# ascentai/diy-gym

Measured on AMD Instinct MI355X. Metric: env steps/sec (whole node), higher is better.
Workload: dtype f32; 1 GPU; ur_high_5 x 16384 envs per GPU; envs_total=16384, substeps=2, auto_reset=True, launch=hipGraph replay of 8-step segments, parallelism=independent env shards x1, no collective, envs_per_wavefront=64, lds_bytes_per_workgroup=160512, parity=vs the C oracle only; parity with pybullet itself is UNPINNED (DESIGN.md 4)

## Files before the change

### diy_gym_amd/csrc/dg_solver.h

```cpp
#pragma once
#include "dg_kernels.h"
#include "dg_hull.h"

namespace dg {

enum { PS_UPDATE = 0, PS_KIN, PS_COLLIDE, PS_ABA, PS_MINV, PS_ROWS, PS_PGS, PS_INTEGRATE, PS_OUTPUT, PS_PGS_MOTOR, PS_PGS_LIMIT, PS_PGS_CONTACT, PS_COUNT,
       PS_ROW = PS_COUNT + 12  };
template <bool PROF> struct Prof;
template <> struct Prof<false> { DGD void start() {} DGD void stamp(int) {} };
template <> struct Prof<true> {
  unsigned long long last, acc[PS_COUNT];
  DGD void start() { _Pragma("unroll") for (int k = 0; k < PS_COUNT; k++) acc[k] = 0ull; last = __builtin_amdgcn_s_memtime(); }
  DGD void stamp(int id) {
    unsigned long long t = __builtin_amdgcn_s_memtime();
    _Pragma("unroll") for (int k = 0; k < PS_COUNT; k++) if (k == id) acc[k] += t - last;
    last = t;
  }
};

struct WShape { int type, body, glink; M3 R; V3 p; float prm0, prm1, prm2, mu; int poff, npts; };

template <int LANES>
DGD void shape_world(const Lane<LANES>& ln, int sh, WShape& o) {
  cip si = ln.sc.SI + sh * DG_SI_STRIDE; cfp sf = ln.sc.SF + sh * DG_SF_STRIDE;
// ... 1657 lines not shown
}

DGD float half_swap_max(float x) {
  float a = x, b = x;
  asm volatile("s_nop 1\n\tv_permlane32_swap_b32 %0, %1" : "+v"(a), "+v"(b));
  return fmaxf(a, b);
}
DGD float half_swap_sum(float x) {
  float a = x, b = x;
  asm volatile("s_nop 1\n\tv_permlane32_swap_b32 %0, %1" : "+v"(a), "+v"(b));
  return a + b;
}
template <int LANES>
DGD void pgs_reg_halves(const Lane<LANES>& ln, int wave) {
  constexpr int RN = 6;
  const DevScene& sc = ln.sc; const float h = sc.h; const float thr_abs = sqrtf(sc.HF[DG_HF_RESIDUAL_THRESHOLD]);
  const int lane = threadIdx.x & 63, half = lane >> 5, el = (lane & 31) + 32 * wave;
  float* const col = ln.lds - lane + el;
  const bool valid = (int)blockIdx.x * 64 + el < sc.num_envs;
  const int b0 = sc.reg_body[0], b1 = sc.helper_body;
  const int f0 = ln.bi(b0)[DG_BI_FIRST_LINK], f1 = ln.bi(b1)[DG_BI_FIRST_LINK], n0 = ln.bi(b0)[DG_BI_N_LINKS], n1 = ln.bi(b1)[DG_BI_N_LINKS];
  const int n = half ? n1 : n0, mvo = half ? ln.plb(b1)[PLB_MINV] : ln.plb(b0)[PLB_MINV], dvo = half ? ln.plb(b1)[PLB_DV] : ln.plb(b0)[PLB_DV];
  const int mo0 = half ? ln.pll(f1)[PLL_MROW] : ln.pll(f0)[PLL_MROW];
  auto W = [&](int slot) -> float& { return col[slot * 64]; };
  float rM[RN * RN], rdv[RN], rb[RN], racc[RN], rdi[RN], rdg[RN], smax[RN], lb[2][RN], la[2][RN]; bool any_limit = false;
  if (n0 == RN && n1 == RN) {
    const float* const cm = col + (size_t)mvo * 64; const float* const cr = col + (size_t)mo0 * 64;
#pragma unroll
    for (int i = 0; i < RN; i++) {
      const float mf0 = ln.mt.v[3 * (f0 + i) + 2], mf1 = ln.mt.v[3 * (f1 + i) + 2], maxf = half ? mf1 : mf0;
      smax[i] = maxf < 0.f ? -maxf : maxf * sc.hm;
#pragma unroll
      for (int c = 0; c < RN; c++) rM[i * RN + c] = cm[(i * RN + c) * 64];
      rb[i] = cr[(i * MR_STRIDE + MR_B) * 64]; rdg[i] = rM[i * RN + i]; rdi[i] = 1.0f / rdg[i];
      lb[0][i] = cr[(i * MR_STRIDE + MR_LO_B) * 64]; la[0][i] = cr[(i * MR_STRIDE + MR_LO_ACC) * 64];
      lb[1][i] = cr[(i * MR_STRIDE + MR_HI_B) * 64]; la[1][i] = cr[(i * MR_STRIDE + MR_HI_ACC) * 64];
      rdv[i] = 0.f; racc[i] = 0.f;
    }
  } else {
#pragma unroll
  for (int i = 0; i < RN; i++) {
    const bool has = i < n; const int ic = has ? i : 0;
    const float mf0 = ln.mt.v[3 * (f0 + (i < n0 ? i : 0)) + 2], mf1 = ln.mt.v[3 * (f1 + (i < n1 ? i : 0)) + 2];
    const float maxf = half ? mf1 : mf0;
    smax[i] = has ? (maxf < 0.f ? -maxf : maxf * sc.hm) : 0.f;
    const int mo = mo0 + ic * MR_STRIDE;
    rb[i] = has ? W(mo + MR_B) : 0.f; rdg[i] = has ? W(mvo + ic * n + ic) : 1.f; rdi[i] = has ? 1.0f / rdg[i] : 0.f;
    lb[0][i] = W(mo + MR_LO_B); la[0][i] = has ? W(mo + MR_LO_ACC) : -1.f;
    lb[1][i] = W(mo + MR_HI_B); la[1][i] = has ? W(mo + MR_HI_ACC) : -1.f;
    any_limit = any_limit || la[0][i] >= 0.f || la[1][i] >= 0.f;
    rdv[i] = 0.f; racc[i] = 0.f;
#pragma unroll
    for (int c = 0; c < RN; c++) { const bool hc = has && c < n; const float m = W(mvo + ic * n + (c < n ? c : 0)); rM[i * RN + c] = hc ? m : 0.f; }
  }
  }
  if (sc.HF[DG_HF_MOTOR_GUESS] > 0.f) chain_motor_guess(rM, rb, smax, racc, rdv, limit_ptol(sc), lb[0], la[0], lb[1], la[1]);
  unsigned lim_rows = 0u;
#pragma unroll
  for (int i = 0; i < RN; i++) { if (__any(la[0][i] >= 0.f)) lim_rows |= 1u << (2 * i); if (__any(la[1][i] >= 0.f)) lim_rows |= 2u << (2 * i); }
  (void)any_limit;
  constexpr int CM = DG_SPLIT_MAX_CONTACTS;
  const int ncont = (int)W(sc.cont_off), g = (half ? ln.plb(b1)[PLB_DV] : ln.plb(b0)[PLB_DV]) - sc.dv_base;
  int cmax = 0;
#pragma unroll
  for (int c = 0; c < CM; c++) if (__any(c < ncont)) cmax = c + 1;
  float cJ[3 * CM][RN], cR[3 * CM][RN], cb[3 * CM], cdg[3 * CM], cdi[3 * CM], cacc[3 * CM], cmu[CM];
  if (cmax > 0) {
    const int nt = sc.nt, rs = sc.crow_tail + 3;
#pragma unroll
    for (int c = 0; c < CM; c++) {
      const bool has = c < ncont; const int cc = has ? c : 0;
      cmu[c] = has ? W(sc.cont_off + 1 + cc * CL_STRIDE + CL_MU) : 0.f;
#pragma unroll
      for (int d = 0; d < 3; d++) {
        const int r = 3 * c + d, ro = sc.tr_off + (3 * cc + d) * rs;
#pragma unroll
        for (int k = 0; k < RN; k++) { const bool hk = has && k < n; const int kk = k < n ? k : 0; const float j = W(ro + g + kk), rr = W(ro + nt + g + kk); cJ[r][k] = hk ? j : 0.f; cR[r][k] = hk ? rr : 0.f; }
        const float bb = W(ro + 2 * nt), dd = W(ro + 2 * nt + 2);
        cb[r] = has ? bb : 0.f; cdg[r] = has ? dd : 1.f; cdi[r] = (has && dd > 1e-18f) ? frcp(dd) : 0.f;
        const float a0 = W(ro + 2 * nt + 1); cacc[r] = (has && cdi[r] != 0.f) ? a0 : 0.f;
#pragma unroll
        for (int k = 0; k < RN; k++) rdv[k] += cR[r][k] * cacc[r];
      }
    }
  }
  bool live = valid; int iters_done = 0;
  auto contact_row = [&](int r, float lo, float hi, float lv, float& maxabs) {
    float jp = 0.f;
#pragma unroll
    for (int k = 0; k < RN; k++) jp += cJ[r][k] * rdv[k];
    const float jv = half_swap_sum(jp);
    const float nacc = fminf(fmaxf(cacc[r] + (cb[r] - jv) * cdi[r], lo), hi);
    const float delta = cdi[r] != 0.f ? (nacc - cacc[r]) * lv : 0.f; cacc[r] += delta;
#pragma unroll
    for (int k = 0; k < RN; k++) rdv[k] += cR[r][k] * delta;
    maxabs = fmaxf(maxabs, fabsf(delta * cdg[r]));
  };
  auto sweep = [&](auto with_limits, auto with_contacts) {
    float maxabs = 0.f; const float lv = live ? 1.f : 0.f;
#pragma unroll
    for (int i = 0; i < RN; i++) {
      const float want = racc[i] + (rb[i] - rdv[i]) * rdi[i];
      const float nacc = __builtin_amdgcn_fmed3f(want, -smax[i], smax[i]);
      const float delta = (nacc - racc[i]) * lv; racc[i] += delta;
#pragma unroll
      for (int c = 0; c < RN; c++) rdv[c] += rM[i * RN + c] * delta;
      maxabs = fmaxf(maxabs, fabsf(delta * rdg[i]));
    }
    if constexpr (decltype(with_limits)::value) {
#pragma unroll
      for (int i = 0; i < RN; i++) {
#pragma unroll
        for (int side = 0; side < 2; side++) {
          if (!((lim_rows >> (2 * i + side)) & 1u)) continue;
          const float sg = side == 0 ? 1.f : -1.f; const bool act = la[side][i] >= 0.f;
          const float nacc = fmaxf(la[side][i] + (lb[side][i] - sg * rdv[i]) * rdi[i], 0.f);
          const float delta = act ? (nacc - la[side][i]) * lv : 0.f; la[side][i] += delta;
          const float sd = sg * delta;
#pragma unroll
          for (int c = 0; c < RN; c++) rdv[c] += rM[i * RN + c] * sd;
          maxabs = fmaxf(maxabs, fabsf(delta * rdg[i]));
        }
      }
    }
    if constexpr (decltype(with_contacts)::value) {
#pragma unroll
      for (int c = 0; c < CM; c++) if (c < cmax) contact_row(3 * c, 0.f, 3.0e38f, lv, maxabs);
#pragma unroll
      for (int c = 0; c < CM; c++) if (c < cmax) {
        const float lim = cmu[c] * cacc[3 * c];
        contact_row(3 * c + 1, -lim, lim, lv, maxabs); contact_row(3 * c + 2, -lim, lim, lv, maxabs);
      }
    }
    const float m = half_swap_max(maxabs);
    live = live && !(m <= thr_abs);
  };
  if (cmax > 0) {
    for (int it = 0; it < sc.iters; it++) { if (live) iters_done = it + 1; sweep(std::true_type{}, std::true_type{}); if (!__any(live)) break; }
  } else if (lim_rows == 0u) {
    for (int it = 0; it < sc.iters; it++) { if (live) iters_done = it + 1; sweep(std::false_type{}, std::false_type{}); if (!__any(live)) break; }
  } else {
    for (int it = 0; it < sc.iters; it++) { if (live) iters_done = it + 1; sweep(std::true_type{}, std::false_type{}); if (!__any(live)) break; }
  }
#pragma unroll
  for (int i = 0; i < RN; i++) if (i < n) { W(dvo + i) = rdv[i]; W(mo0 + i * MR_STRIDE + MR_ACC) = racc[i]; }
  if (cmax > 0 && half == 0) {
    const int rs = sc.crow_tail + 3;
#pragma unroll
    for (int c = 0; c < CM; c++) if (c < ncont) { _Pragma("unroll") for (int d = 0; d < 3; d++) W(sc.tr_off + (3 * c + d) * rs + sc.crow_tail + 1) = cacc[3 * c + d]; }
  }
  if (half == 0) W(split_slots(sc)) = (float)iters_done;
}

template <int LANES, bool PROF, bool PAR = false, bool SLICED = false, bool FULLWAVE = false>
DGD void substep(const Lane<LANES>& ln, int32_t* diag_out, Prof<PROF>& prof, float* smem = nullptr, float* gws = nullptr, int index = 0) {
  const DevScene& sc = ln.sc; const float h = sc.h; const int hb = PAR ? sc.helper_body : -1;
  const bool primary = SLICED ? (int)threadIdx.x < envs_per_wave(LANES) : true;
  constexpr int LCH = 6;
  int ncont = 0, wave_max_cont = 0, iters_done = 0;
  uint64_t limit_mask = 0ull;
  uint64_t limit_rows = 0ull;
  const float thr = sc.HF[DG_HF_RESIDUAL_THRESHOLD]; const int rs = crow_stride(sc.crow_tail);
  const bool early = PAR && sc.early_dyn && index == 0;
  constexpr int EPW = envs_per_wave(LANES), SLN = SLICED ? 64 / EPW : 1, SLOG = SLN == 64 ? 6 : SLN == 16 ? 4 : SLN == 8 ? 3 : SLN == 4 ? 2 : SLN == 2 ? 1 : 0;
  const int qlane = threadIdx.x & 63, qsl = qlane & (SLN - 1), qe = qlane >> SLOG;
  const int qenv = blockIdx.x * EPW + qe; const bool qvalid = qenv < sc.num_envs; const int qec = qvalid ? qenv : sc.num_envs - 1;
  const Lane<LANES> lq(sc, ln.mt, SLICED ? ln.lds - qlane + qe : ln.lds, SLICED ? ln.st - ln.env + qec : ln.st, SLICED ? qec : ln.env, SLICED ? qvalid : ln.valid);
  if (primary) {
  if (index == sc.substeps - 1 && !early) for (int b = 0; b < sc.nba; b++) if (b != hb) save_prev_velocities(ln, b);
  if (!early) for (int b = 0; b < sc.nba; b++) if (b != hb) ln.kinematics(b);
  }
  if (PAR) __syncthreads();
  prof.stamp(PS_KIN);
  if constexpr (SLICED) collide<LANES, 64, SLN>(lq, 0, 0x7fffffff, -1, qsl);
  const bool own_collide = !(PAR && sc.coll_wave);
  if (primary) {
  if constexpr (SLICED) ncont = (int)ln.L(sc.cont_off);
  else if (own_collide) ncont = collide<LANES, FULLWAVE ? 64 : (PAR ? 64 : 0)>(ln);
  prof.stamp(PS_COLLIDE);
  }
  if (!early) for (int b = 0; b < sc.nba; b++) {
    if (b == hb || (ln.fixed(b) && ln.bi(b)[DG_BI_N_LINKS] == 0)) continue;
    const int mslices = (SLICED && !ln.plb(b)[PLB_CHAIN] && !sc.no_minv_slices) ? ln.minv_slices(b, SLN) : 0;
    if (primary) { if (ln.plb(b)[PLB_CHAIN]) ln.template dynamics_chain<6>(b, prof); else ln.dynamics(b, prof, mslices > 0); }
    if constexpr (SLICED) { if (mslices > 0) { lq.minv_sliced(b, qsl, mslices, SLN); prof.stamp(4 ); } }
    if (primary) {
      const int dvo = ln.plb(b)[PLB_DV], nv = ln.plb(b)[PLB_NV];
      for (int k = 0; k < nv; k++) ln.L(dvo + k) = 0.f;
    }
  }
  if (primary) {
  if (PAR) __syncthreads();
  if (!own_collide) {
    ncont = (int)ln.L(sc.cont_off);
    if (sc.coll_split) {
      const int nb2 = (int)ln.L(sc.cont2_off);
      if (__any(nb2 > 0)) {
        for (int j = 0; j < sc.max_contacts; j++) {
          if (!__any(j < nb2)) break;
          if (j < nb2 && ncont + j < sc.max_contacts) {
            float* dst = ln.lds + (sc.cont_off + 1 + (ncont + j) * CL_STRIDE) * envs_per_wave(LANES);
#pragma unroll
            for (int k = 0; k < CL_KEY + 1; k++) dst[k * envs_per_wave(LANES)] = ln.L(sc.cont2_off + 1 + j * CL_STRIDE + k);
          }
        }
        ncont = min(ncont + nb2, sc.max_contacts); ln.L(sc.cont_off) = (float)ncont;
      }
    }
  }
  const bool helper_rows = PAR && sc.split_pgs;
  if (helper_rows) {
    const int hf = ln.bi(hb)[DG_BI_FIRST_LINK], hn = ln.bi(hb)[DG_BI_N_LINKS];
    setup_link_rows(ln, 0, hf, limit_mask, limit_rows); setup_link_rows(ln, hf + hn, sc.nl, limit_mask, limit_rows);
  } else setup_link_rows(ln, 0, sc.nl, limit_mask, limit_rows);
  for (int b = 0; b < sc.nba; b++) {
    if (ln.bi(b)[DG_BI_N_LINKS] == 0 || b == sc.reg_body[0] || b == sc.reg_body[1] || (helper_rows && b == hb)) continue;
    motor_guess(ln, b);
  }
  if (sc.ncons > 0) build_constraint_rows(ln);
  const bool vel_dense = sc.dense && sc.nt >= 1 && sc.reg_body[0] < 0;
  wave_max_cont = [&] { int m = ncont; for (int o = 32; o > 0; o >>= 1) m = max(m, __shfl_xor(m, o)); return m; }();
  if (vel_dense && wave_max_cont > 0)
    for (int b = 0; b < sc.nba; b++) if (!(ln.fixed(b) && ln.bi(b)[DG_BI_N_LINKS] == 0)) ln.gen_vel_store(b, ln.plb(b)[PLB_DV]);
  if constexpr (!SLICED) {
  for (int c = 0; c < wave_max_cont; c++) {
    const bool has = c < ncont; const int mypair = has ? (int)ln.L(sc.cont_off + 1 + c * CL_STRIDE + CL_PAIR) : -1;
    bool todo = has && !build_contact_rows_base(ln, c, has, vel_dense);
    if (!sc.no_chain_rows) todo = todo && !build_contact_rows_chains(ln, c, todo);
    while (__any(todo)) {
      const int leader = __ffsll((long long)__ballot(todo)) - 1;
      const int pair = __shfl(mypair, leader);
      const bool mine = todo && mypair == pair;
      build_contact_rows(ln, c, pair, mine, vel_dense);
      todo = todo && !mine;
    }
  }
  prof.stamp(PS_ROWS);
  }
  }
  if constexpr (SLICED) {
    constexpr int SL = SLN, CPI = SL >= 4 ? SL / 4 : SL;
    const int sl = qsl;
    const int ncq = __shfl(ncont, qe), wmc = __builtin_amdgcn_readfirstlane(wave_max_cont);
    const bool vd = sc.dense && sc.nt >= 1 && sc.reg_body[0] < 0;
    const int csub = SL >= 4 ? sl >> 2 : sl, d_lo = SL >= 4 ? (sl & 3) : 0, d_hi = SL >= 4 ? ((sl & 3) < 3 ? (sl & 3) + 1 : 0) : 3;
    for (int c0 = 0; c0 < wmc; c0 += CPI) {
      const int c = c0 + csub; const bool has = c < ncq && d_lo < d_hi;
      const int mypair = has ? (int)lq.L(sc.cont_off + 1 + c * CL_STRIDE + CL_PAIR) : -1;
      bool todo = has && !build_contact_rows_base(lq, c, has, vd, d_lo, d_hi);
      while (__any(todo)) {
        const int leader = __ffsll((long long)__ballot(todo)) - 1;
        const int pair = __shfl(mypair, leader);
        const bool mine = todo && mypair == pair;
        build_contact_rows(lq, c, pair, mine, vd, d_lo, d_hi);
        todo = todo && !mine;
      }
    }
    prof.stamp(PS_ROWS);
  }
  bool split_now = false;
  if constexpr (PAR) split_now = split_decide_main(ln, wave_max_cont, limit_mask, limit_rows);
  const bool all_dense = sc.dense && sc.nt >= 1 && sc.reg_body[0] < 0;
  if constexpr (SLICED) {
    wave_max_cont = __builtin_amdgcn_readfirstlane(wave_max_cont);
    limit_rows = ((uint64_t)(uint32_t)__builtin_amdgcn_readfirstlane((int)(limit_rows >> 32)) << 32) | (uint32_t)__builtin_amdgcn_readfirstlane((int)(uint32_t)limit_rows);
  }
  if (SLICED && all_dense) {
    const bool try_regs = sc.split_pgs != -1;
    if constexpr (SLICED && LANES == 1) {
      iters_done = pgs_wave_env<PROF>(lq, __builtin_amdgcn_readfirstlane(ncont), limit_rows, prof);
    } else if constexpr (SLICED && LANES == 4) {
      if (sc.nt <= 16) { if (!(try_regs && pgs_sliced_regs_dispatch<LANES, 16, PROF>(ln, ncont, wave_max_cont, limit_rows, prof, iters_done))) iters_done = pgs_dense_sliced<LANES, 16, PROF>(ln, ncont, wave_max_cont, limit_rows, prof); }
      else if (!(try_regs && pgs_sliced_regs_dispatch<LANES, 32, PROF>(ln, ncont, wave_max_cont, limit_rows, prof, iters_done))) iters_done = pgs_dense_sliced<LANES, 32, PROF>(ln, ncont, wave_max_cont, limit_rows, prof);
    } else if constexpr (SLICED && LANES > 0) {
      if (sc.nt <= 8) { if (!(try_regs && pgs_sliced_regs_dispatch<LANES, 8, PROF>(ln, ncont, wave_max_cont, limit_rows, prof, iters_done))) iters_done = pgs_dense_sliced<LANES, 8, PROF>(ln, ncont, wave_max_cont, limit_rows, prof); }
      else if (sc.nt <= 16) { if (!(try_regs && pgs_sliced_regs_dispatch<LANES, 16, PROF>(ln, ncont, wave_max_cont, limit_rows, prof, iters_done))) iters_done = pgs_dense_sliced<LANES, 16, PROF>(ln, ncont, wave_max_cont, limit_rows, prof); }
      else if (sc.nt <= 24) iters_done = pgs_dense_sliced<LANES, 24, PROF>(ln, ncont, wave_max_cont, limit_rows, prof);
      else iters_done = pgs_dense_sliced<LANES, 32, PROF>(ln, ncont, wave_max_cont, limit_rows, prof);
    } else if constexpr (SLICED) {
      if (sc.nt <= 8) iters_done = pgs_dense_sliced_global<LANES, 8, PROF>(ln, smem, gws, ncont, wave_max_cont, limit_rows, prof);
      else if (sc.nt <= 16) iters_done = pgs_dense_sliced_global<LANES, 16, PROF>(ln, smem, gws, ncont, wave_max_cont, limit_rows, prof);
      else if (sc.nt <= 24) iters_done = pgs_dense_sliced_global<LANES, 24, PROF>(ln, smem, gws, ncont, wave_max_cont, limit_rows, prof);
      else iters_done = pgs_dense_sliced_global<LANES, 32, PROF>(ln, smem, gws, ncont, wave_max_cont, limit_rows, prof);
    }
  } else if (PAR && split_now) {
    prof.stamp(PS_PGS_MOTOR);
    pgs_reg_halves(ln, 0);
    prof.stamp(PS_PGS_LIMIT);
    __syncthreads();
    prof.stamp(PS_PGS_CONTACT);
    iters_done = (int)ln.L(split_slots(sc));
  } else if (primary) {
  bool live = ln.valid;
  constexpr bool FW = FULLWAVE || PAR;
  if (all_dense || (sc.dense && (wave_max_cont > 0 || limit_mask != 0ull) && sc.nl <= 32)) {
    for (int k = 0; k < 2; k++) if (sc.reg_body[k] >= 0) motor_guess(ln, sc.reg_body[k]);
    if (sc.nt <= 8) iters_done = pgs_dense<LANES, 8, PROF, FW>(ln, ncont, wave_max_cont, limit_rows, prof);
    else if (sc.nt <= 16) iters_done = pgs_dense<LANES, 16, PROF, FW>(ln, ncont, wave_max_cont, limit_rows, prof);
    else if (sc.nt <= 24) iters_done = pgs_dense<LANES, 24, PROF, FW>(ln, ncont, wave_max_cont, limit_rows, prof);
    else iters_done = pgs_dense<LANES, 32, PROF, FW>(ln, ncont, wave_max_cont, limit_rows, prof);
  } else {
  constexpr int NBR = 2, RN = 6;
  float rM[NBR][RN * RN], rdv[NBR][RN], rb[NBR][RN], racc[NBR][RN], rdi[NBR][RN], rdg[NBR][RN]; float smax[NBR][RN]; int rn[NBR];
#pragma unroll
  for (int k = 0; k < NBR; k++) {
    const int b = sc.reg_body[k]; rn[k] = 0;
#pragma unroll
    for (int i = 0; i < RN; i++) { rdv[k][i] = 0.f; rb[k][i] = 0.f; racc[k][i] = 0.f; rdi[k][i] = 0.f; rdg[k][i] = 0.f; smax[k][i] = 0.f;
      _Pragma("unroll") for (int c = 0; c < RN; c++) rM[k][i * RN + c] = 0.f; }
    if (b >= 0) {
      const int n = ln.bi(b)[DG_BI_N_LINKS], first = ln.bi(b)[DG_BI_FIRST_LINK], mvo = ln.plb(b)[PLB_MINV], mo0 = ln.pll(first)[PLL_MROW];
      rn[k] = n;
#pragma unroll
      for (int i = 0; i < RN; i++) {
        rdv[k][i] = 0.f; rb[k][i] = 0.f; racc[k][i] = 0.f; rdi[k][i] = 0.f; rdg[k][i] = 0.f; smax[k][i] = 0.f;
        if (i < n) {
          const float maxf = ln.mt.v[3 * (first + i) + 2]; smax[k][i] = maxf < 0.f ? -maxf : maxf * sc.hm;
          rb[k][i] = ln.L(mo0 + i * MR_STRIDE + MR_B); rdg[k][i] = ln.L(mvo + i * n + i); rdi[k][i] = 1.0f / rdg[k][i];
        }
#pragma unroll
        for (int c = 0; c < RN; c++) rM[k][i * RN + c] = (i < n && c < n) ? ln.L(mvo + i * n + c) : 0.f;
      }
    }
  }
  auto regs_to_lds = [&](int k) { const int b = sc.reg_body[k]; if (b < 0) return; const int dvo = ln.plb(b)[PLB_DV];
    _Pragma("unroll") for (int i = 0; i < RN; i++) if (i < rn[k]) ln.L(dvo + i) = rdv[k][i]; };
  auto lds_to_regs = [&](int k) { const int b = sc.reg_body[k]; if (b < 0) return; const int dvo = ln.plb(b)[PLB_DV];
    _Pragma("unroll") for (int i = 0; i < RN; i++) if (i < rn[k]) rdv[k][i] = ln.L(dvo + i); };
  bool has_generic = false;
  for (int b = 0; b < sc.nba; b++) if (ln.bi(b)[DG_BI_N_LINKS] > 0 && b != sc.reg_body[0] && b != sc.reg_body[1]) has_generic = true;
  const float thr_abs = sqrtf(thr);
  if (sc.HF[DG_HF_MOTOR_GUESS] > 0.f) {
#pragma unroll
    for (int k = 0; k < NBR; k++) if (sc.reg_body[k] >= 0) {
      const int mo0 = ln.pll(ln.bi(sc.reg_body[k])[DG_BI_FIRST_LINK])[PLL_MROW]; const float ptol = limit_ptol(sc); const bool pinning = ptol >= 0.f;
      float lb0[RN], la0[RN], lb1[RN], la1[RN];
      _Pragma("unroll") for (int i = 0; i < RN; i++) { const bool has = i < rn[k]; const int mo = mo0 + (has ? i : 0) * MR_STRIDE;
        lb0[i] = ln.L(mo + MR_LO_B); la0[i] = has ? ln.L(mo + MR_LO_ACC) : -1.f; lb1[i] = ln.L(mo + MR_HI_B); la1[i] = has ? ln.L(mo + MR_HI_ACC) : -1.f; }
      chain_motor_guess(rM[k], rb[k], smax[k], racc[k], rdv[k], ptol, lb0, la0, lb1, la1);
      if (pinning) { _Pragma("unroll") for (int i = 0; i < RN; i++) if (i < rn[k]) { ln.L(mo0 + i * MR_STRIDE + MR_LO_ACC) = la0[i]; ln.L(mo0 + i * MR_STRIDE + MR_HI_ACC) = la1[i]; } }
    }
    if (has_generic) for (int b = 0; b < sc.nba; b++) {
      const int n = ln.bi(b)[DG_BI_N_LINKS]; if (n == 0 || b == sc.reg_body[0] || b == sc.reg_body[1]) continue;
      const int first = ln.bi(b)[DG_BI_FIRST_LINK], k0 = ln.fixed(b) ? 0 : 6, nv = ln.plb(b)[PLB_NV], dvo = ln.plb(b)[PLB_DV], mvo = ln.plb(b)[PLB_MINV];
      for (int i = 0; i < n; i++) { const int mo = ln.pll(first + i)[PLL_MROW]; const float a0 = ln.L(mo + MR_ACC) + fmaxf(ln.L(mo + MR_LO_ACC), 0.f) - fmaxf(ln.L(mo + MR_HI_ACC), 0.f); lds_axpy(ln, dvo, mvo + (k0 + i) * nv, a0, nv); }
    }
  }
  if (wave_max_cont > 0 && sc.warm_off >= 0) {
    const int nvm = sc.nv_max; const bool two = sc.crow_tail > 2 * nvm;
    regs_to_lds(0); regs_to_lds(1);
    for (int c = 0; c < wave_max_cont; c++) {
      const bool has = c < ncont; const int co = sc.cont_off + 1 + c * CL_STRIDE;
#pragma unroll
      for (int d = 0; d < 3; d++) {
        const int ro = sc.tr_off + (3 * c + d) * rs; const float a0 = has ? ln.L(ro + sc.crow_tail + 1) : 0.f;
        if (a0 != 0.f) {
          lds_axpy(ln, (int)ln.L(co + CL_DVA), ro + nvm, a0, nvm);
          if (two && (int)ln.L(co + CL_NVB) > 0) lds_axpy(ln, (int)ln.L(co + CL_DVB), ro + 3 * nvm, a0, nvm);
        }
      }
    }
    lds_to_regs(0); lds_to_regs(1);
  }
  for (int it = 0; it < sc.iters; it++) {
    float maxres = 0.f, maxabs = 0.f;
    {
      const float lv = live ? 1.f : 0.f;
#pragma unroll
      for (int i = 0; i < RN; i++) {
#pragma unroll
        for (int k = 0; k < NBR; k++) {
          const float want = racc[k][i] + (rb[k][i] - rdv[k][i]) * rdi[k][i];
          const float nacc = __builtin_amdgcn_fmed3f(want, -smax[k][i], smax[k][i]);
          const float delta = (nacc - racc[k][i]) * lv; racc[k][i] += delta;
#pragma unroll
          for (int c = 0; c < RN; c++) rdv[k][c] += rM[k][i * RN + c] * delta;
          maxabs = fmaxf(maxabs, fabsf(delta * rdg[k][i]));
        }
      }
    }
    if (has_generic) for (int b = 0; b < sc.nba; b++) {
      const int n = ln.bi(b)[DG_BI_N_LINKS]; if (n == 0 || b == sc.reg_body[0] || b == sc.reg_body[1]) continue;
      if (ln.fixed(b) && n <= 8) maxres = fmaxf(maxres, pgs_rows_small<LANES, 8, false>(ln, b, live));
      else maxres = fmaxf(maxres, pgs_rows_generic<LANES, false>(ln, b, live));
    }
    prof.stamp(PS_PGS_MOTOR);
    if (limit_mask) {
      for (int b = 0; b < sc.nba; b++) {
        const int n = ln.bi(b)[DG_BI_N_LINKS]; if (n == 0 || !((limit_mask >> (b & 63)) & 1ull)) continue;
        if (b == sc.reg_body[0]) regs_to_lds(0);
        if (b == sc.reg_body[1]) regs_to_lds(1);
        if (ln.fixed(b) && n <= 8) maxres = fmaxf(maxres, pgs_rows_small<LANES, 8, true>(ln, b, live));
        else maxres = fmaxf(maxres, pgs_rows_generic<LANES, true>(ln, b, live));
        if (b == sc.reg_body[0]) lds_to_regs(0);
        if (b == sc.reg_body[1]) lds_to_regs(1);
      }
    }
    prof.stamp(PS_PGS_LIMIT);
    if (wave_max_cont > 0 || sc.ncons > 0) { regs_to_lds(0); regs_to_lds(1); }
    for (int q = 0; q < sc.ncons; q++) {
      const float lim = sc.KF[q * DG_KF_STRIDE + DG_KF_MAX_FORCE] * h;
      for (int d = 0; d < 6; d++) {
        const int c = sc.max_contacts + 2 * q + d / 3;
        maxres = fmaxf(maxres, solve_crow(ln, sc.tr_off + (3 * c + d % 3) * rs, sc.cont_off + 1 + c * CL_STRIDE, -lim, lim, live, true));
      }
    }
    {
    for (int c = 0; c < wave_max_cont; c++) {
      const bool has = c < ncont;
      float r = solve_crow(ln, sc.tr_off + (3 * c) * rs, sc.cont_off + 1 + c * CL_STRIDE, 0.f, 3.0e38f, live, has);
      if (has) maxres = fmaxf(maxres, r);
    }
    for (int c = 0; c < wave_max_cont; c++) {
      const bool has = c < ncont;
      const float mu = has ? ln.L(sc.cont_off + 1 + c * CL_STRIDE + CL_MU) : 0.f;
      const bool act = has && mu > 0.f;
      const float lim = act ? mu * ln.L(sc.tr_off + (3 * c) * rs + sc.crow_tail + 1) : 0.f;
#pragma unroll
      for (int d = 1; d < 3; d++) { float r = solve_crow(ln, sc.tr_off + (3 * c + d) * rs, sc.cont_off + 1 + c * CL_STRIDE, -lim, lim, live, act); if (act) maxres = fmaxf(maxres, r); }
    }
    }
    if (wave_max_cont > 0 || sc.ncons > 0) { lds_to_regs(0); lds_to_regs(1); }
    prof.stamp(PS_PGS_CONTACT);
    if (live) iters_done = it + 1;
    live = live && !(maxres <= thr && maxabs <= thr_abs);
    if (!__any(live)) break;
  }
#pragma unroll
  for (int k = 0; k < NBR; k++) {
    const int b = sc.reg_body[k];
    if (b >= 0) {
      regs_to_lds(k);
      const int mo0 = ln.pll(ln.bi(b)[DG_BI_FIRST_LINK])[PLL_MROW];
#pragma unroll
      for (int i = 0; i < RN; i++) if (i < rn[k]) ln.L(mo0 + i * MR_STRIDE + MR_ACC) = racc[k][i];
    }
  }
  }
  }
  prof.stamp(PS_PGS);
  if (primary) {
  store_warm_cache(ln, ncont, wave_max_cont);
  if (diag_out && ln.valid) {
    int32_t* d = diag_out + (size_t)DG_DIAG_STRIDE * ln.env;
    d[DG_DIAG_CONTACTS] = ncont; d[DG_DIAG_PGS_ITERS] = iters_done;
    if (index == 0) { d[DG_DIAG_PGS_ITERS_FIRST] = iters_done; d[DG_DIAG_CONTACTS_FIRST] = ncont; }
  }
  for (int b = 0; b < sc.nba; b++) if (!(split_now && b == hb)) integrate_body(ln, b);
  }
  if (PAR) __syncthreads();
}

template <int LANES>
DGD void helper_substep(const Lane<LANES>& ln, bool early, bool last) {
  const DevScene& sc = ln.sc; const int hb = sc.helper_body; Prof<false> none;
  if (last && !early) save_prev_velocities(ln, hb);
  if (!early) ln.kinematics(hb);
  __syncthreads();
  if (!early) {
    ln.template dynamics_chain<6>(hb, none);
    const int dvo = ln.plb(hb)[PLB_DV], nv = ln.plb(hb)[PLB_NV]; for (int k = 0; k < nv; k++) ln.L(dvo + k) = 0.f;
  }
  __syncthreads();
  uint64_t lm = 0ull, lr = 0ull;
  if (sc.split_pgs) { const int hf = ln.bi(hb)[DG_BI_FIRST_LINK]; setup_link_rows(ln, hf, hf + ln.bi(hb)[DG_BI_N_LINKS], lm, lr); }
  const int hf0 = ln.bi(hb)[DG_BI_FIRST_LINK];
  if (split_decide_follow(ln, hf0 + 6 <= 32 ? (unsigned)((lr >> (2 * hf0)) & 0xFFFull) : 0u, true)) {
    pgs_reg_halves(ln, 1);
    __syncthreads();
    integrate_body(ln, hb);
  }
  __syncthreads();
}

template <int LANES, bool PROF, bool PAR = false, bool SLICED = false, bool FULLWAVE = false>
DGD void sim_step(const Lane<LANES>& ln, int32_t* diag_out, Prof<PROF>& prof, float* smem = nullptr, float* gws = nullptr) {
  const DevScene& sc = ln.sc;
  for (int k = 0; k < sc.substeps; k++) { substep<LANES, PROF, PAR, SLICED, FULLWAVE>(ln, diag_out, prof, smem, gws, k); prof.stamp(PS_INTEGRATE); }
  if (SLICED && (int)threadIdx.x >= envs_per_wave(LANES)) return;
  if (sc.debug_keep_ext) return;
  for (int b = 0; b < sc.nba; b++) { if (ln.frozen(b)) continue; const int eo = ln.ext_off(b); for (int k = 0; k < 6; k++) ln.Sset(eo + k, 0.f); }
  for (int gl = 0; gl < sc.nl; gl++) ln.Sset(ln.li(gl)[DG_LI_STATE_OFF] + DG_LS_TORQUE, 0.f);
}

template <int LANES>
DGD int run_ik(const Lane<LANES>& ln, int op, const float* act, bool live_lane) {
  const DevScene& sc = ln.sc; cip oi = sc.OI + op * DG_OI_STRIDE;
  const int b = oi[DG_OI_BODY], fr = oi[DG_OI_FRAME], flags = oi[DG_OI_FLAGS];
  const bool use_orn = flags & DG_IK_USE_ORIENTATION, nullsp = flags & DG_IK_NULLSPACE;
  const int first = ln.bi(b)[DG_BI_FIRST_LINK], n = ln.bi(b)[DG_BI_N_LINKS];
  const int qo = sc.tr_off, jo = qo + n, vo = jo + 6 * n, dto = vo + n;
  cfp rest = sc.FL + oi[DG_OI_FLIST];
  for (int i = 0; i < n; i++) ln.L(qo + i) = ln.S(ln.li(first + i)[DG_LI_STATE_OFF] + DG_LS_Q);
  V3 cp, cv, cw; Q4 cq; ln.frame_state(b, fr, true, cp, cq, cv, cw, false);
  V3 tp = cp + v3(act[0], act[1], act[2]); Q4 tq = cq;
  if (use_orn) tq = qmul(cq, qfrom_euler(act[3], act[4], act[5]));
  const int eel = sc.FI[fr * DG_FI_STRIDE + DG_FI_LINK];
  const float lam2 = nullsp ? sc.HF[DG_HF_IK_LAMBDA_SQ] : sc.HF[DG_HF_IK_JOINT_DAMPING], maxang = sc.HF[DG_HF_IK_MAX_ANGLE], g0 = sc.HF[DG_HF_IK_NULL_REST_GAIN], g1 = sc.HF[DG_HF_IK_NULL_LIMIT_GAIN];
  const float resid = sc.HF[DG_HF_IK_RESIDUAL];
  bool live = live_lane; int iters = 0;
  for (int it = 0; it < sc.ik_iters; it++) {
    ln.kinematics(b, qo);
    V3 fp, fv, fw; Q4 fq; ln.frame_state(b, fr, true, fp, fq, fv, fw, false);
    V3 ep = tp - fp;
    if (it > 0 && norm(ep) < resid) live = false;
    if (!__any(live)) break;
    iters += live ? 1 : 0;
    float dS[6] = {ep.x, ep.y, ep.z, 0.f, 0.f, 0.f};
    if (use_orn) {
      Q4 dq = qmul(tq, qconj(fq)); if (dq.w < 0.f) { dq.x = -dq.x; dq.y = -dq.y; dq.z = -dq.z; dq.w = -dq.w; }
      float sn = sqrtf(dq.x * dq.x + dq.y * dq.y + dq.z * dq.z), an = 2.0f * atan2f(sn, dq.w), k = sn > 1e-12f ? an / sn : 2.0f;
      dS[3] = dq.x * k; dS[4] = dq.y * k; dS[5] = dq.z * k;
    }
    for (int i = 0; i < 6 * n; i++) ln.L(jo + i) = 0.f;
    for (int k = eel; k >= 0; k = ln.li(k)[DG_LI_PARENT]) {
      int po = ln.pll(k)[PLL_POSE]; M3 Rk = ln.LR(po); V3 pk = ln.L3(po + 6); cfp f = ln.lf(k);
      V3 axw = mul(Rk, v3(f[DG_LF_AXIS], f[DG_LF_AXIS + 1], f[DG_LF_AXIS + 2])); int i = k - first;
      V3 jl, ja; if (ln.li(k)[DG_LI_TYPE] == 0) { jl = cross(axw, fp - pk); ja = axw; } else { jl = axw; ja = v3(0, 0, 0); }
      ln.L(jo + i) = jl.x; ln.L(jo + n + i) = jl.y; ln.L(jo + 2 * n + i) = jl.z;
      if (use_orn) { ln.L(jo + 3 * n + i) = ja.x; ln.L(jo + 4 * n + i) = ja.y; ln.L(jo + 5 * n + i) = ja.z; }
    }
    float U[21];
#pragma unroll
    for (int k = 0; k < 21; k++) U[k] = 0.f;
    for (int k = 0; k < n; k++) {
      float col[6];
#pragma unroll
      for (int r = 0; r < 6; r++) col[r] = ln.L(jo + r * n + k);
#pragma unroll
      for (int r = 0; r < 6; r++)
#pragma unroll
        for (int c = 0; c <= r; c++) U[r * (r + 1) / 2 + c] += col[r] * col[c];
    }
#pragma unroll
    for (int r = 0; r < 6; r++) U[r * (r + 1) / 2 + r] += lam2;
    chol6(U);
    float y[6]; chol6_solve(U, dS, y);
    float Jv[6] = {0.f, 0.f, 0.f, 0.f, 0.f, 0.f};
    for (int k = 0; k < n; k++) {
      float t = 0.f;
#pragma unroll
      for (int r = 0; r < 6; r++) t += ln.L(jo + r * n + k) * y[r];
      float v0 = 0.f;
      if (nullsp) {
        float q = ln.L(qo + k), lo = rest[n + k], hi = rest[2 * n + k], rg = rest[3 * n + k];
        v0 = g0 * (rest[k] - q);
        if (q > hi) v0 += g1 * (hi - q) / rg;
        if (q < lo) v0 += g1 * (lo - q) / rg;
#pragma unroll
        for (int r = 0; r < 6; r++) Jv[r] += ln.L(jo + r * n + k) * v0;
      }
      ln.L(vo + k) = v0; ln.L(dto + k) = t;
    }
    float mx = 0.f;
    if (nullsp) {
      float z[6]; chol6_solve(U, Jv, z);
      for (int k = 0; k < n; k++) {
        float t = 0.f;
#pragma unroll
        for (int r = 0; r < 6; r++) t += ln.L(jo + r * n + k) * z[r];
        float d = ln.L(dto + k) + ln.L(vo + k) - t; ln.L(dto + k) = d; mx = fmaxf(mx, fabsf(d));
      }
    } else {
      for (int k = 0; k < n; k++) mx = fmaxf(mx, fabsf(ln.L(dto + k)));
    }
    const float scl = mx > maxang ? maxang / mx : 1.0f;
    for (int k = 0; k < n; k++) if (live) ln.L(qo + k) += scl * ln.L(dto + k);
  }
  return iters;
}

#define DG_IK_DEV_CHAIN 256
#define DG_IK_DEV_FULL 512
template <int LANES, int N, bool FULL = false, bool NS = false, bool ORN = false>
DGD int run_ik_chain(const Lane<LANES>& ln, int op, const float* act, bool live_lane, float* qout) {
  const DevScene& sc = ln.sc; cip oi = sc.OI + op * DG_OI_STRIDE;
  const int b = oi[DG_OI_BODY], fr = oi[DG_OI_FRAME], flags = oi[DG_OI_FLAGS];
  const bool use_orn = FULL ? ORN : (flags & DG_IK_USE_ORIENTATION) != 0, nullsp = FULL ? NS : (flags & DG_IK_NULLSPACE) != 0;
  const int first = ln.bi(b)[DG_BI_FIRST_LINK], n = FULL ? N : ln.bi(b)[DG_BI_N_LINKS];
  const int eel = FULL ? N - 1 : sc.FI[fr * DG_FI_STRIDE + DG_FI_LINK] - first;
  cfp rest = sc.FL + oi[DG_OI_FLIST]; cfp ff = sc.FF + fr * DG_FF_STRIDE;
  const V3 off = v3(ff[DG_FF_COM_POS], ff[DG_FF_COM_POS + 1], ff[DG_FF_COM_POS + 2]);
  const Q4 qoff = {ff[DG_FF_COM_QUAT], ff[DG_FF_COM_QUAT + 1], ff[DG_FF_COM_QUAT + 2], ff[DG_FF_COM_QUAT + 3]};
  const M3 R0 = ln.LR(ln.plb(b)[PLB_R0]); const V3 p0 = ln.base_pos(b);
  float q[N]; V3 ow[N], aw[N];
  float cR[N][9], cP[N][3]; bool rev[N];
  M3 Qprev = {{1.f, 0.f, 0.f, 0.f, 1.f, 0.f, 0.f, 0.f, 1.f}}, Qee = Qprev;
#pragma unroll
  for (int i = 0; i < N; i++) {
    q[i] = 0.f; rev[i] = true;
#pragma unroll
    for (int k = 0; k < 9; k++) cR[i][k] = 0.f;
#pragma unroll
    for (int k = 0; k < 3; k++) cP[i][k] = 0.f;
    if (FULL || i < n) {
      cfp f = ln.lf(first + i); q[i] = ln.S(ln.li(first + i)[DG_LI_STATE_OFF] + DG_LS_Q); rev[i] = FULL || ln.li(first + i)[DG_LI_TYPE] == 0;
      M3 RT; _Pragma("unroll") for (int k = 0; k < 9; k++) RT.m[k] = pin(f[DG_LF_ROT + k]);
      const V3 pT = v3(pin(f[DG_LF_POS]), pin(f[DG_LF_POS + 1]), pin(f[DG_LF_POS + 2]));
      const V3 ax = v3(pin(f[DG_LF_AXIS]), pin(f[DG_LF_AXIS + 1]), pin(f[DG_LF_AXIS + 2]));
      V3 u, v; tangent_basis(ax, u, v);
      const M3 Qi = {{u.x, v.x, ax.x, u.y, v.y, ax.y, u.z, v.z, ax.z}};
      const M3 RTp = mul(transpose(Qprev), mul(RT, Qi)); const V3 pTp = tmul(Qprev, pT);
#pragma unroll
      for (int k = 0; k < 9; k++) cR[i][k] = RTp.m[k];
      cP[i][0] = pTp.x; cP[i][1] = pTp.y; cP[i][2] = pTp.z;
      Qprev = Qi; if (FULL ? i == N - 1 : i == eel) Qee = Qi;
    }
  }
  const V3 offp = tmul(Qee, off);
  float nRest[N], nLo[N], nHi[N], nIrg[N];
#pragma unroll
  for (int i = 0; i < N; i++) {
    nRest[i] = 0.f; nLo[i] = -3.0e38f; nHi[i] = 3.0e38f; nIrg[i] = 0.f;
    if (nullsp && (FULL || i < n)) { nRest[i] = pin(rest[i]); nLo[i] = pin(rest[n + i]); nHi[i] = pin(rest[2 * n + i]); nIrg[i] = pin(frcp(rest[3 * n + i])); }
  }
  V3 pe; M3 Re;
// ... 612 lines not shown
```

### diy_gym_amd/csrc/dg_step_par_body.inc

```
  constexpr int reset_mode = DG_PAR_RESET;
  extern __shared__ float smem[];
  const int wave = threadIdx.x >> 6, lane = threadIdx.x & 63;
  const int env = blockIdx.x * 64 + lane; const bool exists = env < sc.num_envs; const int e = exists ? env : sc.num_envs - 1;
  const bool doit = exists && (!reset_mode || reset_mask == nullptr || reset_mask[e] != 0);
  if (reset_mode && !__any(doit)) return;
  const bool valid = reset_mode ? doit : exists;
  const float* act_row = actions ? actions + (size_t)e * sc.act_dim : nullptr;
  const unsigned long long t_start = PROF ? __builtin_amdgcn_s_memtime() : 0ull; (void)t_start;
  if (wave == 3) {
    Lane<64> ln(sc, mt, smem + lane, state + e, e, valid);
    if (reset_mode) __syncthreads();
    DG_WAVE_STAMP(0); __syncthreads();
    if (sc.early_dyn) {
      early_dynamics(ln, 1);
      if (sc.coll_split) collide<64, 64>(ln, sc.npairs / 2, 0x7fffffff, sc.cont2_off);
    }
    DG_WAVE_STAMP(1); __syncthreads();
    for (int k = 0; k < sc.substeps; k++) {
      __syncthreads();
      if (sc.coll_split && !(sc.early_dyn && k == 0)) collide<64, 64>(ln, sc.npairs / 2, 0x7fffffff, sc.cont2_off);
      __syncthreads();
      if (split_decide_follow(ln, 0u, false)) __syncthreads();
      __syncthreads();
    }
    DG_WAVE_STAMP(2); __syncthreads();
    run_output_ops(ln, nullptr, (valid && rew) ? rew + (size_t)e * sc.rew_dim : nullptr, (valid && term) ? term + (size_t)e * sc.term_dim : nullptr,
                   (valid && rew_sum) ? rew_sum + e : nullptr, (valid && term_flag) ? term_flag + e : nullptr, OUT_REW_TERM);
    DG_WAVE_STAMP(3);
    return;
  }
  if (wave == 2) {
    Lane<64> ln(sc, mt, smem + lane, state + e, e, valid);
    if (reset_mode) __syncthreads();
    DG_WAVE_STAMP(0); __syncthreads();
    if (sc.early_dyn) {
      collide<64, 64>(ln, 0, sc.coll_split ? sc.npairs / 2 : 0x7fffffff);
      early_dynamics(ln, 0);
    }
    DG_WAVE_STAMP(1); __syncthreads();
    for (int k = 0; k < sc.substeps; k++) {
      __syncthreads();
      if (sc.coll_wave && !(sc.early_dyn && k == 0)) collide<64, 64>(ln, 0, sc.coll_split ? sc.npairs / 2 : 0x7fffffff);
      __syncthreads();
      if (split_decide_follow(ln, false, false)) __syncthreads();
      __syncthreads();
    }
    DG_WAVE_STAMP(2); __syncthreads();
    run_output_ops(ln, (valid && obs) ? obs + (size_t)e * sc.obs_dim : nullptr, nullptr, nullptr, nullptr, nullptr, OUT_OBS_REST);
    DG_WAVE_STAMP(3);
    return;
  }
  if (wave == 1) {
    Lane<64> ln(sc, mt, smem + lane, state + e, e, valid);
    if (reset_mode) __syncthreads();
    ln.kinematics(sc.helper_body);
    DG_WAVE_STAMP(0); __syncthreads();
    if (act_row) run_update_ops(ln, act_row, mask, sc.helper_body, -1, diag);
    DG_WAVE_STAMP(1); __syncthreads();
    for (int k = 0; k < sc.substeps; k++) helper_substep(ln, sc.early_dyn && k == 0, k == sc.substeps - 1);
    ln.kinematics(sc.helper_body);
    DG_WAVE_STAMP(2); __syncthreads();
    run_output_ops(ln, (valid && obs) ? obs + (size_t)e * sc.obs_dim : nullptr, nullptr, nullptr, nullptr, nullptr, OUT_JOINT_OF, sc.helper_body);
    DG_WAVE_STAMP(3);
    return;
  }
  Lane<64> ln(sc, mt, smem + lane, state + e, e, valid);
  Prof<PROF> prof; prof.start();
  if (reset_mode) { if (doit) { ln.Sset(DG_ST_STEP, 0.0f); run_reset_ops(ln); } __syncthreads(); }
  for (int b = 0; b < sc.nba; b++) if (b != sc.helper_body) ln.kinematics(b);
  __syncthreads();
  prof.stamp(PS_KIN);
  if (act_row) run_update_ops(ln, act_row, mask, -1, sc.helper_body, diag);
  if (!reset_mode) ln.Sset(DG_ST_STEP, ln.S(DG_ST_STEP) + 1.0f);
  __syncthreads();
  prof.stamp(PS_UPDATE);
  sim_step<64, PROF, true>(ln, diag, prof);
  for (int b = 0; b < sc.nba; b++) if (b != sc.helper_body) ln.kinematics(b);
  __syncthreads();
  prof.stamp(PS_KIN);
  run_output_ops(ln, (valid && obs) ? obs + (size_t)e * sc.obs_dim : nullptr, nullptr, nullptr, nullptr, nullptr, OUT_JOINT_NOT_OF, sc.helper_body);
  prof.stamp(PS_OUTPUT);
  if constexpr (PROF) { if (lane == 0) for (int k = 0; k < PS_COUNT; k++) cycles[(size_t)blockIdx.x * PS_ROW + k] = prof.acc[k]; }
```

Measured before the change: 170.4 million env-steps/s.

## Add fused contact-free joint PGS path split across two waves by half

When no contacts exist in a wave and both arms are 6-link chains with no constraints, the main and helper waves skip row building, split decisions and the generic PGS. Each wave instead solves 32 envs, one arm per half-wave, with an in-register 6x6 motor/limit PGS, then integrates joint state directly to global memory. This is meant to remove contact-row setup, split synchronisation and generic solver overhead in contact-free substeps. It adds a second code path with its own integration and diagnostics handling, and it relies on every wave agreeing on the contact-free predicate so the barrier counts still match.

```diff
diff --git a/diy_gym_amd/csrc/dg_solver.h b/diy_gym_amd/csrc/dg_solver.h
--- a/diy_gym_amd/csrc/dg_solver.h
+++ b/diy_gym_amd/csrc/dg_solver.h
@@ -1833,12 +1833,117 @@
   if (half == 0) W(split_slots(sc)) = (float)iters_done;
 }
 
+template <int LANES>
+DGD bool substep_contact_free(const Lane<LANES>& ln) {
+  const DevScene& sc = ln.sc;
+  if (sc.split_pgs <= 0 || sc.ncons > 0) return false;
+  if (ln.bi(sc.reg_body[0])[DG_BI_N_LINKS] != 6 || ln.bi(sc.helper_body)[DG_BI_N_LINKS] != 6) return false;
+  float cnt = ln.L(sc.cont_off);
+  if (sc.coll_split) cnt = fmaxf(cnt, ln.L(sc.cont2_off));
+  return !__any(cnt > 0.f);
+}
+template <int LANES, bool PROF>
+DGD void fused_free_halves(const Lane<LANES>& ln, int wave, Prof<PROF>& prof) {
+  constexpr int RN = 6;
+  const DevScene& sc = ln.sc; const float h = sc.h, lerp = sc.HF[DG_HF_LIMIT_ERP], vmax = sc.HF[DG_HF_MAX_COORD_VEL];
+  const float thr_abs = sqrtf(sc.HF[DG_HF_RESIDUAL_THRESHOLD]);
+  int lane = threadIdx.x & 63; asm volatile("" : "+v"(lane));
+  const int half = lane >> 5, el = (lane & 31) + 32 * wave;
+  float* const col = ln.lds - (threadIdx.x & 63) + el;
+  const int envl = (int)blockIdx.x * 64 + el; const bool exists = envl < sc.num_envs;
+  const bool store = (__ballot(ln.valid) >> el) & 1ull;
+  float* const st = ln.st - ln.env + (exists ? envl : sc.num_envs - 1);
+  const size_t stride = sc.stride;
+  const int b0 = sc.reg_body[0], b1 = sc.helper_body;
+  const int f0 = ln.bi(b0)[DG_BI_FIRST_LINK], f1 = ln.bi(b1)[DG_BI_FIRST_LINK];
+  const int mvo = half ? ln.plb(b1)[PLB_MINV] : ln.plb(b0)[PLB_MINV];
+  const float* const cm = col + (size_t)mvo * 64;
+  int lo[RN]; float q[RN], qd[RN], tp[RN], tv[RN];
+#pragma unroll
+  for (int i = 0; i < RN; i++) {
+    const int lo0 = ln.li(f0 + i)[DG_LI_STATE_OFF], lo1 = ln.li(f1 + i)[DG_LI_STATE_OFF]; lo[i] = half ? lo1 : lo0;
+    q[i] = st[(lo[i] + DG_LS_Q) * stride]; qd[i] = st[(lo[i] + DG_LS_QD) * stride];
+    tp[i] = st[(lo[i] + DG_LS_TARGET_POS) * stride]; tv[i] = st[(lo[i] + DG_LS_TARGET_VEL) * stride];
+  }
+  float rM[RN * RN], rdv[RN], rb[RN], racc[RN], rdi[RN], rdg[RN], smax[RN], lb[2][RN], la[2][RN];
+#pragma unroll
+  for (int i = 0; i < RN; i++) {
+#pragma unroll
+    for (int c = 0; c < RN; c++) rM[i * RN + c] = cm[(i * RN + c) * 64];
+    rdg[i] = rM[i * RN + i]; rdi[i] = 1.0f / rdg[i]; rdv[i] = 0.f; racc[i] = 0.f;
+  }
+#pragma unroll
+  for (int i = 0; i < RN; i++) {
+    const float* m0 = ln.mt.v + 3 * (f0 + i); const float* m1 = ln.mt.v + 3 * (f1 + i); cfp fa = ln.lf(f0 + i), fb = ln.lf(f1 + i);
+    const float kp = half ? m1[0] : m0[0], kd = half ? m1[1] : m0[1], maxf = half ? m1[2] : m0[2];
+    const float lower = half ? fb[DG_LF_LOWER] : fa[DG_LF_LOWER], upper = half ? fb[DG_LF_UPPER] : fa[DG_LF_UPPER];
+    smax[i] = maxf < 0.f ? -maxf : maxf * sc.hm;
+    rb[i] = kp * (tp[i] - q[i]) / h + kd * (tv[i] - qd[i]);
+    const bool limited = lower <= upper;
+    const float dlo = q[i] - lower, dhi = upper - q[i];
+    lb[0][i] = -qd[i] + (dlo > 0.f ? -dlo / h : -dlo * lerp / h); la[0][i] = (limited && dlo < 0.25f) ? 0.f : -1.f;
+    lb[1][i] = qd[i] + (dhi > 0.f ? -dhi / h : -dhi * lerp / h); la[1][i] = (limited && dhi < 0.25f) ? 0.f : -1.f;
+  }
+  prof.stamp(PS_ROWS);
+  if (sc.HF[DG_HF_MOTOR_GUESS] > 0.f) chain_motor_guess(rM, rb, smax, racc, rdv, limit_ptol(sc), lb[0], la[0], lb[1], la[1]);
+  unsigned lim_rows = 0u;
+#pragma unroll
+  for (int i = 0; i < RN; i++) { if (__any(la[0][i] >= 0.f)) lim_rows |= 1u << (2 * i); if (__any(la[1][i] >= 0.f)) lim_rows |= 2u << (2 * i); }
+  bool live = exists; int iters_done = 0;
+  auto sweep = [&](auto with_limits) {
+    float maxabs = 0.f; const float lv = live ? 1.f : 0.f;
+#pragma unroll
+    for (int i = 0; i < RN; i++) {
+      const float want = racc[i] + (rb[i] - rdv[i]) * rdi[i];
+      const float nacc = __builtin_amdgcn_fmed3f(want, -smax[i], smax[i]);
+      const float delta = (nacc - racc[i]) * lv; racc[i] += delta;
+#pragma unroll
+      for (int c = 0; c < RN; c++) rdv[c] += rM[i * RN + c] * delta;
+      maxabs = fmaxf(maxabs, fabsf(delta * rdg[i]));
+    }
+    if constexpr (decltype(with_limits)::value) {
+#pragma unroll
+      for (int i = 0; i < RN; i++) {
+#pragma unroll
+        for (int side = 0; side < 2; side++) {
+          if (!((lim_rows >> (2 * i + side)) & 1u)) continue;
+          const float sg = side == 0 ? 1.f : -1.f; const bool act = la[side][i] >= 0.f;
+          const float nacc = fmaxf(la[side][i] + (lb[side][i] - sg * rdv[i]) * rdi[i], 0.f);
+          const float delta = act ? (nacc - la[side][i]) * lv : 0.f; la[side][i] += delta;
+          const float sd = sg * delta;
+#pragma unroll
+          for (int c = 0; c < RN; c++) rdv[c] += rM[i * RN + c] * sd;
+          maxabs = fmaxf(maxabs, fabsf(delta * rdg[i]));
+        }
+      }
+    }
+    const float m = half_swap_max(maxabs);
+    live = live && !(m <= thr_abs);
+  };
+  if (lim_rows == 0u) {
+    for (int it = 0; it < sc.iters; it++) { if (live) iters_done = it + 1; sweep(std::false_type{}); if (!__any(live)) break; }
+  } else {
+    for (int it = 0; it < sc.iters; it++) { if (live) iters_done = it + 1; sweep(std::true_type{}); if (!__any(live)) break; }
+  }
+  prof.stamp(PS_PGS_LIMIT);
+  if (store) {
+#pragma unroll
+    for (int i = 0; i < RN; i++) {
+      st[(lo[i] + DG_LS_APPLIED) * stride] = smax[i] > 0.f ? racc[i] / h : 0.f;
+      const float qn = fminf(fmaxf(qd[i] + rdv[i], -vmax), vmax);
+      st[(lo[i] + DG_LS_QD) * stride] = qn; st[(lo[i] + DG_LS_Q) * stride] = q[i] + h * qn;
+    }
+  }
+  if (half == 0) col[split_slots(sc) * 64] = (float)iters_done;
+}
+
 template <int LANES, bool PROF, bool PAR = false, bool SLICED = false, bool FULLWAVE = false>
 DGD void substep(const Lane<LANES>& ln, int32_t* diag_out, Prof<PROF>& prof, float* smem = nullptr, float* gws = nullptr, int index = 0) {
   const DevScene& sc = ln.sc; const float h = sc.h; const int hb = PAR ? sc.helper_body : -1;
   const bool primary = SLICED ? (int)threadIdx.x < envs_per_wave(LANES) : true;
   constexpr int LCH = 6;
   int ncont = 0, wave_max_cont = 0, iters_done = 0;
+  bool fused = false;
   uint64_t limit_mask = 0ull;
   uint64_t limit_rows = 0ull;
   const float thr = sc.HF[DG_HF_RESIDUAL_THRESHOLD]; const int rs = crow_stride(sc.crow_tail);
@@ -1872,6 +1977,8 @@
   }
   if (primary) {
   if (PAR) __syncthreads();
+  if constexpr (PAR) { fused = substep_contact_free(ln); if (fused) fused_free_halves(ln, 0, prof); }
+  if (!fused) {
   if (!own_collide) {
     ncont = (int)ln.L(sc.cont_off);
     if (sc.coll_split) {
@@ -1919,6 +2026,7 @@
   prof.stamp(PS_ROWS);
   }
   }
+  }
   if constexpr (SLICED) {
     constexpr int SL = SLN, CPI = SL >= 4 ? SL / 4 : SL;
     const int sl = qsl;
@@ -1940,13 +2048,14 @@
     prof.stamp(PS_ROWS);
   }
   bool split_now = false;
-  if constexpr (PAR) split_now = split_decide_main(ln, wave_max_cont, limit_mask, limit_rows);
+  if constexpr (PAR) { if (!fused) split_now = split_decide_main(ln, wave_max_cont, limit_mask, limit_rows); }
   const bool all_dense = sc.dense && sc.nt >= 1 && sc.reg_body[0] < 0;
   if constexpr (SLICED) {
     wave_max_cont = __builtin_amdgcn_readfirstlane(wave_max_cont);
     limit_rows = ((uint64_t)(uint32_t)__builtin_amdgcn_readfirstlane((int)(limit_rows >> 32)) << 32) | (uint32_t)__builtin_amdgcn_readfirstlane((int)(uint32_t)limit_rows);
   }
-  if (SLICED && all_dense) {
+  if (PAR && fused) {
+  } else if (SLICED && all_dense) {
     const bool try_regs = sc.split_pgs != -1;
     if constexpr (SLICED && LANES == 1) {
       iters_done = pgs_wave_env<PROF>(lq, __builtin_amdgcn_readfirstlane(ncont), limit_rows, prof);
@@ -2120,16 +2229,20 @@
   }
   }
   prof.stamp(PS_PGS);
-  if (primary) {
-  store_warm_cache(ln, ncont, wave_max_cont);
-  if (diag_out && ln.valid) {
+  auto write_diag = [&] {
     int32_t* d = diag_out + (size_t)DG_DIAG_STRIDE * ln.env;
     d[DG_DIAG_CONTACTS] = ncont; d[DG_DIAG_PGS_ITERS] = iters_done;
     if (index == 0) { d[DG_DIAG_PGS_ITERS_FIRST] = iters_done; d[DG_DIAG_CONTACTS_FIRST] = ncont; }
-  }
-  for (int b = 0; b < sc.nba; b++) if (!(split_now && b == hb)) integrate_body(ln, b);
+  };
+  if (primary) {
+  store_warm_cache(ln, ncont, wave_max_cont);
+  if (diag_out && ln.valid && !fused) write_diag();
+  for (int b = 0; b < sc.nba; b++) if (!((split_now || fused) && b == hb) && !(fused && b == sc.reg_body[0])) integrate_body(ln, b);
   }
   if (PAR) __syncthreads();
+  if constexpr (PAR) {
+    if (fused && diag_out && ln.valid) { iters_done = (int)ln.L(split_slots(sc)); write_diag(); }
+  }
 }
 
 template <int LANES>
@@ -2143,6 +2256,7 @@
     const int dvo = ln.plb(hb)[PLB_DV], nv = ln.plb(hb)[PLB_NV]; for (int k = 0; k < nv; k++) ln.L(dvo + k) = 0.f;
   }
   __syncthreads();
+  if (substep_contact_free(ln)) { fused_free_halves(ln, 1, none); __syncthreads();  return; }
   uint64_t lm = 0ull, lr = 0ull;
   if (sc.split_pgs) { const int hf = ln.bi(hb)[DG_BI_FIRST_LINK]; setup_link_rows(ln, hf, hf + ln.bi(hb)[DG_BI_N_LINKS], lm, lr); }
   const int hf0 = ln.bi(hb)[DG_BI_FIRST_LINK];
diff --git a/diy_gym_amd/csrc/dg_step_par_body.inc b/diy_gym_amd/csrc/dg_step_par_body.inc
--- a/diy_gym_amd/csrc/dg_step_par_body.inc
+++ b/diy_gym_amd/csrc/dg_step_par_body.inc
@@ -20,7 +20,7 @@
       __syncthreads();
       if (sc.coll_split && !(sc.early_dyn && k == 0)) collide<64, 64>(ln, sc.npairs / 2, 0x7fffffff, sc.cont2_off);
       __syncthreads();
-      if (split_decide_follow(ln, 0u, false)) __syncthreads();
+      if (!substep_contact_free(ln) && split_decide_follow(ln, 0u, false)) __syncthreads();
       __syncthreads();
     }
     DG_WAVE_STAMP(2); __syncthreads();
@@ -42,7 +42,7 @@
       __syncthreads();
       if (sc.coll_wave && !(sc.early_dyn && k == 0)) collide<64, 64>(ln, 0, sc.coll_split ? sc.npairs / 2 : 0x7fffffff);
       __syncthreads();
-      if (split_decide_follow(ln, false, false)) __syncthreads();
+      if (!substep_contact_free(ln) && split_decide_follow(ln, false, false)) __syncthreads();
       __syncthreads();
     }
     DG_WAVE_STAMP(2); __syncthreads();
```

New measurement: 182.5 million env-steps/s, median of 6. 7.1% higher.
